# vliu15/speech-masters-thesis

Hardware: AMD Instinct MI355X
Metric: LJSpeech utterances/sec per VQ-VAE train step (higher is better)
Workload: dtype bf16

## Files before the change

include/smt_hip.h:

```cpp
#ifndef SMT_HIP_H
#define SMT_HIP_H

#include <stddef.h>
#include <stdint.h>

#ifdef __cplusplus
extern "C" {
#endif

typedef void* smt_stream_t;

enum { SMT_F32 = 0, SMT_BF16 = 1 };

const char* smt_last_error(void);
int smt_abi_version(void);

size_t smt_vq_prep_bytes(int k_bins, int dim);
int smt_vq_prepare(const float* codebook, int k_bins, int dim, void* prep, size_t prep_bytes, smt_stream_t stream);

size_t smt_vq_forward_workspace_bytes(int64_t n_rows, int k_bins, int dim);
int smt_vq_forward(const float* x, const float* codebook, void* prep, const float* row_mask,
                   int64_t n_rows, int k_bins, int dim,
                   int64_t* idx, float* min_dist, float* x_d, float* sums,
                   void* workspace, size_t workspace_bytes, smt_stream_t stream);
// ... 93 lines not shown
  int64_t bs_x, bs_y, bs_res, bs_act, bs_yact;
  const void* x; const void* w; const float* bias; void* y; void* y_act;
  const void* res; const void* act_grad_src;
  const int* lens_in; const int* lens_out;
  int w_swizzled;
  const void* zero_page;
  const void* x2; const void* w2;
  const float* bias2;
  const int* lens_in2;
  int c_in2, ld_x2;
  int64_t bs_x2;
  const uint32_t* drop_keys_dev;
  int drop_keys_dev_stride;
} smt_conv_desc;
int smt_conv1d_ntc(const smt_conv_desc* desc, smt_stream_t stream);
const char* smt_conv1d_kernel_name(const smt_conv_desc* desc);

size_t smt_conv1d_wgrad_workspace_bytes(const smt_conv_desc* desc);
int smt_conv1d_wgrad(const smt_conv_desc* desc, float* dweight, int64_t stride_out, int64_t stride_in,
                     int64_t stride_tap, const int* tap_map, float* dbias, void* workspace,
                     size_t workspace_bytes, smt_stream_t stream);
int smt_wgrad_reduce_defer(int on, smt_stream_t stream);
const char* smt_conv1d_wgrad_kernel_name(const smt_conv_desc* desc);

size_t smt_conv1x1_bwd_workspace_bytes(const smt_conv_desc* desc);
int smt_conv1x1_bwd(const smt_conv_desc* desc, float* dweight, int64_t stride_out, int64_t stride_in, float* dbias,
                    void* workspace, size_t workspace_bytes, smt_stream_t stream);

size_t smt_conv_k1_bwd_workspace_bytes(int batch, int t);
int smt_conv_k1_bwd(const void* dh, int64_t bs_dh, int ld_dh, const void* x, int64_t bs_x, int ld_x,
                    const void* w_packed_bwd, const void* res, int64_t bs_res, int ld_res, void* dx, int64_t bs_dx,
                    int ld_dx, const int* lens, int batch, int t, const void* zero_page, float* dweight,
                    int64_t stride_out, int64_t stride_in, float* dbias, void* workspace, size_t workspace_bytes,
                    smt_stream_t stream);

int smt_convt4s2(const void* x, int64_t bs_x, int ld_x, const void* w_packed, const float* bias, void* y, int64_t bs_y,
                 int ld_y, const int* lens_in, const int* lens_out, int batch, int t_in, int c_out, const void* zero_page,
                 smt_stream_t stream);
int smt_conv4s2(const void* x, int64_t bs_x, int ld_x, const void* w_packed, const float* bias, void* y, int64_t bs_y,
                int ld_y, const int* lens_in, const int* lens_out, int batch, int t_in, int c_in, const void* zero_page,
                smt_stream_t stream);

int smt_conv_k3gate_fwd(const void* u2, int64_t bs_u2, int ld_u2, const void* x, int64_t bs_x, int ld_x,
                        const void* w3_packed, const void* w1_packed, const float* b3, const float* b1, void* z,
                        int64_t bs_z, int ld_z, void* g, int64_t bs_g, int ld_g, const int* lens, int batch, int t,
                        const void* zero_page, smt_stream_t stream);
// ... 167 lines not shown
```

speech-masters-thesis_amd/csrc/conv_wgrad.hip:

```cpp
#include <algorithm>
#include <cstdlib>

#include "conv_common.h"

namespace smt {

struct WgradArgs {
  const void* x; const void* dy; float* slab;
  const int* lens_in;
  long long x_bs, dy_bs;
  int ldx, ldy;
  int B, Tin, Tout, Ty, Cin, Cout;
  int taps, stride, dil, pad, out_stride, out_offset;
  int rows_per_chunk, chunks_per_batch, nblk_ci, nblk_co, with_bias;
};

template <typename T> struct WTr;
template <> struct WTr<__bf16> {
  static constexpr int R = 128;
  static constexpr int pitch(int ch) { return ch + 32; }
};
template <> struct WTr<float> {
  static constexpr int R = 64;
  static constexpr int pitch(int ch) { return ch + 4; }
// ... 254 lines not shown
          const bf16x8 bfrag = tr_read2(xbase + xoff[j] + k0 * XB, 4 * XB);
          acc[j] = __builtin_amdgcn_mfma_f32_32x32x16_bf16(a, bfrag, acc[j], 0, 0, 0);
        } else if (j == ntaps && bias_plane) {
          acc[j] = __builtin_amdgcn_mfma_f32_32x32x16_bf16(a, ones, acc[j], 0, 0, 0);
        }
      }
    }
    step_end_wait<0>();
  }
  const int planes = ntaps + 1;
  float* out = p.slab + ((size_t)w.cgl * w.nblk + w.blk) * (size_t)planes * CB * CIB;
#pragma unroll
  for (int j = 0; j < NT; ++j) {
    if (j >= planes) break;
#pragma unroll
    for (int e = 0; e < 16; ++e) {
      const int row = wm * 32 + (e & 3) + 8 * (e >> 2) + 4 * hh;
      const int col = wn * 32 + r;
      out[((size_t)j * CB + row) * CIB + col] = acc[j][e];
    }
  }
}

struct ShiftArgs {
  const void* x; const void* dy; float* slab; const int* lens_in;
  long long x_bs, dy_bs;
  int ldx, ldy;
  int B, Tin, Tout, pad, rs;
  int tiles_per_item, tiles_per_wg, n_chunks, nblk_ci, nblk_co, with_bias;
};

#ifndef SMT_WGRAD_STAMP
#define SMT_WGRAD_STAMP 0
#endif
#if SMT_WGRAD_STAMP
__device__ unsigned long long wg_dbg[256 * 8 * 8];
__device__ __forceinline__ unsigned long long wg_stamp() {
  unsigned long long t;
  __builtin_amdgcn_sched_barrier(0);
  asm volatile("s_memtime %0\n\ts_waitcnt lgkmcnt(0)" : "=s"(t) : : "memory");
  __builtin_amdgcn_sched_barrier(0);
  return t;
}
#define WG_SUMS unsigned long long wg_sum[5] = {0, 0, 0, 0, 0}
#define WG_T(var) const unsigned long long var = wg_stamp()
#define WG_ACC(k, a, b) wg_sum[k] += (b) - (a)
#define WG_DUMP do { if (lane == 0 && blockIdx.x < 256) for (int k_ = 0; k_ < 5; ++k_) wg_dbg[(blockIdx.x * 8 + wave) * 8 + k_] += wg_sum[k_]; } while (0)
#else
#define WG_SUMS do {} while (0)
#define WG_T(var) do {} while (0)
#define WG_ACC(k, a, b) do {} while (0)
#define WG_DUMP do {} while (0)
#endif

constexpr int SH_R = 128, SH_XROWS = SH_R + 8, SH_DY = SH_R * 128, SH_X = SH_XROWS * 256, SH_STAGE = SH_DY + SH_X;

template <int NTAPS>
__global__ __launch_bounds__(512) void conv_wgrad_shift_kernel(ShiftArgs p, const __bf16* __restrict__ zero_page) {
  constexpr int CB = 64, CIB = 128, WNC = 4, DYB = CB * 2, XB = CIB * 2, PLANES = NTAPS + 1;
  extern __shared__ __attribute__((aligned(16))) unsigned char smem[];
  const int tid = threadIdx.x, lane = tid & 63;
  const int wave = __builtin_amdgcn_readfirstlane(tid >> 6);
  const int wm = wave / WNC, wn = wave % WNC;
  const int r = lane & 31, hh = lane >> 5;

  const WgBlock w = wgrad_block(p.nblk_ci, p.nblk_co);
  if (w.cgl >= p.n_chunks) return;
  const int co0 = (w.blk / p.nblk_ci) * CB, ci0 = (w.blk % p.nblk_ci) * CIB;
  const int ntiles = p.tiles_per_item * p.B * p.rs;
  const int tile_begin = w.cgl * p.tiles_per_wg;
  const int tile_end = min(ntiles, tile_begin + p.tiles_per_wg);
  const int rs = p.rs;
  const bool bias_plane = p.with_bias && (ci0 == 0);

  f32x16 acc[PLANES];
#pragma unroll
  for (int j = 0; j < PLANES; ++j)
#pragma unroll
    for (int e = 0; e < 16; ++e) acc[j][e] = 0.f;

  constexpr int SH_PIECES = 7;
  constexpr int SH_PPS = 2;
  static_assert(SH_PPS <= NTAPS && SH_PPS * (SH_R / 16) >= SH_PIECES, "the pieces fit the k-loop");
  const unsigned pdy = (unsigned)p.ldy * rs * 2u, pxx = (unsigned)p.ldx * rs * 2u;
  const int dyrow = 8 * wave + (lane >> 3), xrow = 4 * wave + (lane >> 4);
  const unsigned voff_dy = (unsigned)dyrow * pdy + (unsigned)(((lane & 7) ^ swz_dy(dyrow)) << 4);
  const unsigned voff_x = (unsigned)xrow * pxx + (unsigned)(((lane & 15) ^ swz_x(xrow)) << 4);
  const unsigned voff_x6 = (128 + xrow < SH_R + NTAPS - 1) ? voff_x + 128u * pxx : 0x80000000u;
  struct Src { __amdgpu_buffer_rsrc_t rdy, rxx; unsigned sdy, sx; };
  auto item_source = [&](int item, Src& s) {
    const int b = item / rs, cls = item - b * rs;
    const int Tc = (p.Tout - cls + rs - 1) / rs;
    const int len_full = p.lens_in ? min(scalar_load_i32(p.lens_in + b), p.Tin) : p.Tin;
    const int len_in = max(0, (len_full - cls + rs - 1) / rs);
    s.rdy = ws_rsrc(p.dy, ((long long)b * p.dy_bs + (long long)cls * p.ldy + co0) * 2, (unsigned)Tc * pdy);
    s.rxx = ws_rsrc(p.x, ((long long)b * p.x_bs + (long long)cls * p.ldx + ci0) * 2, (unsigned)len_in * pxx);
  };
  auto tile_source = [&](int t0, Src& s) {
    s.sdy = (unsigned)t0 * pdy;
    s.sx = (unsigned)(t0 - p.pad) * pxx;
  };
  auto piece = [&](const Src& s, int i, int buf) {
    unsigned char* base = smem + (size_t)buf * SH_STAGE;
    if (i < 2) ws_dma16(s.rdy, voff_dy + s.sdy + (unsigned)(64 * i) * pdy, base + (wave + 8 * i) * 1024);
    else if (i < 6) ws_dma16(s.rxx, voff_x + s.sx + (unsigned)(32 * (i - 2)) * pxx, base + SH_DY + (wave + 8 * (i - 2)) * 1024);
    else if (wave < 2) ws_dma16(s.rxx, voff_x6 + s.sx, base + SH_DY + (wave + 32) * 1024);
  };

  bf16x8 ones;
#pragma unroll
  for (int e = 0; e < 8; ++e) ones[e] = (__bf16)1.0f;

  const int tg = lane >> 4, tq = (lane & 15) >> 2, tp = lane & 3, thh = tg >> 1;
  const int coly = wm * 32 + 16 * (tg & 1) + 4 * tp, colx = wn * 32 + 16 * (tg & 1) + 4 * tp;
  const int lrow = 8 * thh + tq;
  const int dyoff = lrow * DYB + (((coly >> 3) ^ (((lrow >> 1) & 1) << 2)) << 4) + (coly & 7) * 2;
  const int xoff = SH_DY + lrow * XB + (((colx >> 3) ^ ((lrow & 3) << 2)) << 4) + (colx & 7) * 2;
  typedef unsigned u32x4 __attribute__((ext_vector_type(4)));
  typedef unsigned u32x2 __attribute__((ext_vector_type(2)));
// ... 34 lines not shown
      if (more) item_source(n_item, sn);
    }
    if (!more) sn.rdy = sn.rxx = ws_rsrc(p.x, 0, 0);
    tile_source(n_t0, sn);
    WG_T(c2);
    const unsigned base = lds0 + (unsigned)buf * SH_STAGE;
    Frags fr[2];
    request(fr[0], base, 0);
#pragma unroll
    for (int k0 = 0; k0 < SH_R / 16; ++k0) {
      Frags& f = fr[k0 & 1];
      if (k0 + 1 < SH_R / 16) {
        request(fr[(k0 + 1) & 1], base, k0 + 1);
        lgkm_wait<SH_NREAD>(f.a0, f.a1, f.p0, f.p1, f.q0, f.q1);
      } else {
        lgkm_wait<0>(f.a0, f.a1, f.p0, f.p1, f.q0, f.q1);
      }
      const u32x4 aw = {f.a0[0], f.a0[1], f.a1[0], f.a1[1]};
      const bf16x8 a = __builtin_bit_cast(bf16x8, aw);
      const unsigned w[8] = {f.p0[0], f.p0[1], f.p1[0], f.p1[1], f.q0[0], f.q0[1], f.q1[0], f.q1[1]};
#pragma unroll
      for (int s = 0; s < NTAPS; ++s) {
        const int m = s >> 1;
        u32x4 bw;
        if (s & 1) {
#pragma unroll
          for (int i = 0; i < 4; ++i) bw[i] = __builtin_amdgcn_alignbit(w[m + i + 1], w[m + i], 16);
        } else {
          bw = u32x4{w[m], w[m + 1], w[m + 2], w[m + 3]};
        }
        acc[s] = __builtin_amdgcn_mfma_f32_32x32x16_bf16(a, __builtin_bit_cast(bf16x8, bw), acc[s], 0, 0, 0);
        if (s < SH_PPS && SH_PPS * k0 + s < SH_PIECES) {
          __builtin_amdgcn_sched_barrier(0);
          piece(sn, SH_PPS * k0 + s, buf ^ 1);
          __builtin_amdgcn_sched_barrier(0);
        }
      }
      if (bias_plane && (k0 & 3) == wn) acc[NTAPS] = __builtin_amdgcn_mfma_f32_32x32x16_bf16(a, ones, acc[NTAPS], 0, 0, 0);
    }
    WG_T(c3);
    WG_ACC(0, c0, c1); WG_ACC(1, c1, c2); WG_ACC(2, c2, c3); WG_ACC(4, c0, c0 + 1);
  }
  vm_wait<0>();
  WG_T(c4);
  float* out = p.slab + ((size_t)w.cgl * w.nblk + w.blk) * (size_t)PLANES * CB * CIB;
#pragma unroll
  for (int j = 0; j < PLANES; ++j)
#pragma unroll
    for (int e = 0; e < 16; ++e) {
      const int row = wm * 32 + (e & 3) + 8 * (e >> 2) + 4 * hh;
      out[((size_t)j * CB + row) * CIB + wn * 32 + r] = acc[j][e];
    }
  WG_T(c5);
  WG_ACC(3, c4, c5);
  WG_DUMP;
}

struct ShiftPlan { int rs, pad, tiles_per_item, tiles_per_wg, n_chunks, nblk_co, nblk_ci; };
static bool wgrad_shift_plan(const smt_conv_desc* d, ShiftPlan* pl) {
  static const bool off = getenv("SMT_WGRAD_NO_SHIFT") != nullptr;
  if (off || d->dtype != SMT_BF16 || d->stride != 1 || d->out_stride != 1 || d->out_offset != 0 || !d->zero_page ||
      d->c_in % 128 != 0 || d->c_out % 64 != 0 || d->taps < 3 || d->taps > 9 || !(d->taps & 1) || d->t_in != d->t_out)
    return false;
  int rs = 1, pad = d->padding;
  if (d->dilation > 1) {
    if (d->padding % d->dilation != 0 || d->t_out / d->dilation < class_min_rows()) return false;
    rs = d->dilation; pad = d->padding / d->dilation;
  }
  if (pad < 0 || pad > d->taps - 1) return false;
  const long long tc_max = (d->t_out + rs - 1) / rs;
  const long long span = (tc_max + 2 * SH_R) * rs * 2;
  if (span * d->ld_x >= (1ll << 31) || span * d->ld_y >= (1ll << 31)) return false;
  const int tpi = (int)((tc_max + SH_R - 1) / SH_R);
  const long long ntiles = (long long)tpi * d->batch * rs;
  static const int min_tiles = getenv("SMT_SHIFT_MIN_TILES") ? atoi(getenv("SMT_SHIFT_MIN_TILES")) : 256;
  if (ntiles < min_tiles) return false;
  const int nco = d->c_out / 64, nci = d->c_in / 128;
  static const int min_tpw = getenv("SMT_SHIFT_MIN_TPW") ? atoi(getenv("SMT_SHIFT_MIN_TPW")) : 2;
  const long long chunks_target =
      std::max<long long>(8, std::min<long long>(256 / (nco * nci), ntiles / std::max(1, min_tpw)));
  const int tpw = (int)((ntiles + chunks_target - 1) / chunks_target);
  pl->rs = rs; pl->pad = pad; pl->tiles_per_item = tpi; pl->tiles_per_wg = tpw;
  pl->n_chunks = (int)((ntiles + tpw - 1) / tpw); pl->nblk_co = nco; pl->nblk_ci = nci;
  return true;
}

struct WreduceJob {
  const float* slab; float* dw; float* db;
  long long so, si, sj;
  int n_chunks, nblk, nblk_ci, planes, taps, Cin, Cout, cib, bias_cols;
  int block0;
  int wblocks;
  signed char jmap[16];
};
constexpr int WR_MAXJ = 16;
struct WreduceBatch { int n_jobs, total_blocks; WreduceJob job[WR_MAXJ]; };

__global__ __launch_bounds__(256) void conv_wgrad_reduce_kernel(WreduceBatch bt) {
  __shared__ f32x4 part[4][64];
  int j = 0;
#pragma unroll 1
  for (int k = 1; k < bt.n_jobs; ++k)
    if ((int)blockIdx.x >= bt.job[k].block0) j = k;
  const WreduceJob& p = bt.job[j];
  const int lb = blockIdx.x - p.block0;
  const size_t blk_elems = (size_t)p.planes * 64 * p.cib;
  const size_t cstride = (size_t)p.nblk * blk_elems;
// ... 222 lines not shown
  SMT_CHECK_ARG(d && tap_map, "smt_conv1d_wgrad: null pointer");
  SMT_CHECK_ARG(d->taps >= 1 && d->taps <= WG_MAX_TAPS, "smt_conv1d_wgrad: taps must be in [1, 16]");
  SMT_CHECK_ARG(d->x && d->y && dweight && workspace, "smt_conv1d_wgrad: null pointer");
  SMT_CHECK_ARG(d->dtype == SMT_BF16 || d->dtype == SMT_F32, "smt_conv1d_wgrad: bad dtype");
  const bool bf = d->dtype == SMT_BF16;
  const int epv = bf ? 8 : 4;
  SMT_CHECK_ARG(d->c_in % epv == 0 && d->c_out % epv == 0 && d->ld_x % epv == 0 && d->ld_y % epv == 0,
                "smt_conv1d_wgrad: channels / pitches must keep 16-byte alignment");
  WgradPlan pl;
  wgrad_plan(d, &pl);
  SMT_CHECK_ARG(workspace_bytes >= pl.ws_bytes, "smt_conv1d_wgrad: workspace too small");
  const bool empty = d->batch <= 0 || d->t_out <= 0;
  for (int i = 0; i < pl.n; ++i) {
    const WgradLaunch& l = pl.l[i];
    float* slab = reinterpret_cast<float*>((char*)workspace + l.ws_off);
    float* db = i == 0 ? dbias : nullptr;
    if (l.variant == WG_SHIFT) {
      ShiftArgs a;
      a.x = d->x; a.dy = d->y; a.slab = slab; a.lens_in = d->lens_in;
      a.x_bs = d->bs_x; a.dy_bs = d->bs_y; a.ldx = d->ld_x; a.ldy = d->ld_y;
      a.B = d->batch; a.Tin = d->t_in; a.Tout = d->t_out; a.pad = l.pad; a.rs = pl.sh.rs;
      a.tiles_per_item = pl.sh.tiles_per_item; a.tiles_per_wg = pl.sh.tiles_per_wg; a.n_chunks = l.n_chunks;
      a.nblk_ci = l.nblk_ci; a.nblk_co = l.nblk_co; a.with_bias = db ? 1 : 0;
      const __bf16* zp = (const __bf16*)d->zero_page;
      switch (d->taps) {
        case 3: launch_lds(conv_wgrad_shift_kernel<3>, l.grid, 512, l.lds, stream, a, zp); break;
        case 5: launch_lds(conv_wgrad_shift_kernel<5>, l.grid, 512, l.lds, stream, a, zp); break;
        case 7: launch_lds(conv_wgrad_shift_kernel<7>, l.grid, 512, l.lds, stream, a, zp); break;
        default: launch_lds(conv_wgrad_shift_kernel<9>, l.grid, 512, l.lds, stream, a, zp); break;
      }
      SMT_CHECK_LAUNCH(kWgradName[l.variant]);
    } else if (!empty) {
      SMT_CHECK_ARG(l.lds <= WG_MAX_LDS, "conv_wgrad: tile needs %zu B of LDS", l.lds);
      WgradArgs a;
      a.x = d->x; a.dy = d->y; a.slab = slab; a.lens_in = d->lens_in;
      a.x_bs = d->bs_x; a.dy_bs = d->bs_y; a.ldx = d->ld_x; a.ldy = d->ld_y;
      a.B = d->batch; a.Tin = d->t_in; a.Tout = d->t_out; a.Ty = d->t_y; a.Cin = d->c_in; a.Cout = d->c_out;
      a.taps = l.taps; a.stride = d->stride; a.dil = d->dilation; a.pad = l.pad;
      a.out_stride = d->out_stride; a.out_offset = d->out_offset;
      a.rows_per_chunk = l.rows_per_chunk; a.chunks_per_batch = l.chunks_per_batch;
      a.nblk_ci = l.nblk_ci; a.nblk_co = l.nblk_co; a.with_bias = db ? 1 : 0;
      const bool strided = d->stride > 1;
      const int planes = l.taps + 1;
      const WgradKernel k = l.variant == WG_DMA ? dma_kernel(planes)
                          : bf && l.cib == 128  ? generic_kernel<__bf16, 128, false>(planes)
                          : bf ? (strided ? generic_kernel<__bf16, 64, true>(planes) : generic_kernel<__bf16, 64, false>(planes))
                               : (strided ? generic_kernel<float, 64, true>(planes) : generic_kernel<float, 64, false>(planes));
      launch_lds(k, l.grid, l.variant == WG_DMA ? 512 : l.cib * 4, l.lds, stream, a);
      SMT_CHECK_LAUNCH(kWgradName[l.variant]);
    }
    const int bias_cols = l.variant == WG_SHIFT ? 4 : 1;
    int rc = launch_wgrad_reduce(slab, dweight, db, empty ? 0 : l.n_chunks, l.nblk_co, l.nblk_ci, l.taps, d->c_in, d->c_out,
                                 l.cib, stride_out, stride_in, stride_tap, tap_map + l.j0, stream, bias_cols);
    if (rc) return rc;
  }
  return 0;
}
```

speech-masters-thesis_amd/smt_amd/convops.py:

```python
import contextlib
import ctypes
import os
from dataclasses import dataclass

import torch

from . import native as N
from . import packing
from . import profiler
from .packing import Part

SMT_F32, SMT_BF16 = 0, 1
_DT = {torch.float32: SMT_F32, torch.bfloat16: SMT_BF16}


class ConvDesc(ctypes.Structure):
    _fields_ = [("dtype", ctypes.c_int), ("batch", ctypes.c_int), ("t_in", ctypes.c_int), ("t_out", ctypes.c_int),
                ("t_y", ctypes.c_int), ("c_in", ctypes.c_int), ("c_out", ctypes.c_int), ("taps", ctypes.c_int),
                ("stride", ctypes.c_int), ("dilation", ctypes.c_int), ("padding", ctypes.c_int),
                ("out_stride", ctypes.c_int), ("out_offset", ctypes.c_int), ("act_out", ctypes.c_int),
                ("act_grad", ctypes.c_int), ("site_width", ctypes.c_int), ("ld_x", ctypes.c_int),
                ("ld_y", ctypes.c_int), ("ld_res", ctypes.c_int), ("ld_act", ctypes.c_int), ("ld_yact", ctypes.c_int),
                ("drop_keys", ctypes.c_uint32 * 8), ("drop_thresh16", ctypes.c_uint32), ("drop_scale", ctypes.c_float),
                ("bs_x", ctypes.c_int64), ("bs_y", ctypes.c_int64), ("bs_res", ctypes.c_int64),
                ("bs_act", ctypes.c_int64), ("bs_yact", ctypes.c_int64), ("x", ctypes.c_void_p), ("w", ctypes.c_void_p),
                ("bias", ctypes.c_void_p), ("y", ctypes.c_void_p), ("y_act", ctypes.c_void_p), ("res", ctypes.c_void_p),
                ("act_grad_src", ctypes.c_void_p), ("lens_in", ctypes.c_void_p), ("lens_out", ctypes.c_void_p),
                ("w_swizzled", ctypes.c_int), ("zero_page", ctypes.c_void_p),
                ("x2", ctypes.c_void_p), ("w2", ctypes.c_void_p), ("bias2", ctypes.c_void_p),
                ("lens_in2", ctypes.c_void_p), ("c_in2", ctypes.c_int), ("ld_x2", ctypes.c_int),
                ("bs_x2", ctypes.c_int64), ("drop_keys_dev", ctypes.c_void_p), ("drop_keys_dev_stride", ctypes.c_int)]


@dataclass
class DropSpec:
    p: float
    training: bool
    seed: int = 0
    site: int = 0

    def params(self):
        if not self.training or self.p <= 0.0:
            return 0, 0, 1.0
        return dropout_key(self.seed, self.site), int(round(self.p * 65536.0)), 1.0 / (1.0 - self.p)


def _fmix32(h):
    h &= 0xFFFFFFFF
    h ^= h >> 16
    h = (h * 0x85EBCA6B) & 0xFFFFFFFF
    h ^= h >> 13
    h = (h * 0xC2B2AE35) & 0xFFFFFFFF
    h ^= h >> 16
    return h


# ... 23 lines not shown
    key = (device.type, device.index)
    if key not in _zero_pages:
        _zero_pages[key] = torch.zeros(4096, dtype=torch.uint8, device=device)
    return _zero_pages[key]


def _dma_ok(dtype, c_in, c_out):
    return dtype == torch.bfloat16 and c_in % 128 == 0 and c_out % 128 == 0


def _phases(kernel, stride, padding):
    out = []
    for ph in range(stride):
        taps = [(j, (ph + padding - j) // stride) for j in range(kernel) if (ph + padding - j) % stride == 0]
        taps.sort(key=lambda jt: jt[1])
        offs = [o for _, o in taps]
        assert offs == list(range(offs[0], offs[0] + len(offs))), "phase taps must touch consecutive rows"
        out.append(([j for j, _ in taps], -offs[0]))
    return out


_K3GATE = not bool(int(os.environ.get("SMT_NO_K3GATE", "0")))
_RESAMPLE = not bool(int(os.environ.get("SMT_NO_RESAMPLE", "0")))


def _pack(weight, dtype, n_out, n_in, s_out, s_in, s_tap, tap_map, swizzle=False):
    return packing.pack([Part.dense(weight, n_out, n_in, s_out, s_in, s_tap, tap_map, swizzle)], dtype,
                        (len(tap_map), n_out, n_in))


def _pack_fwd(weight, dtype, swizzle=False):
    c_out, c_in, k = weight.shape
    return _pack(weight, dtype, c_out, c_in, c_in * k, k, 1, range(k), swizzle)


def _pack_bwd(weight, dtype, swizzle=False):
    c_out, c_in, k = weight.shape
    return _pack(weight, dtype, c_in, c_out, k, c_in * k, 1, range(k - 1, -1, -1), swizzle)


def _pack_cat_fwd(weights, dtype, swizzle=False):
    n_in = weights[0].shape[1]
    total = sum(w.shape[0] for w in weights)
    parts, row0 = [], 0
    for w in weights:
        parts.append(Part(w, w.shape[0], n_in, n_in, 1, 1, (0,), bool(swizzle), row0 * n_in, total * n_in, n_in))
# ... 71 lines not shown
    d.batch, d.t_in, d.t_out, d.t_y = x.shape[0], x.shape[1], t_out, (y.shape[1] if t_y is None else t_y)
    d.c_in, d.c_out = c_in, c_out
    d.taps, d.stride, d.dilation, d.padding = taps, stride, dil, pad
    d.out_stride, d.out_offset = out_stride, out_offset
    d.x, d.bs_x, d.ld_x = _geom(x)
    if y is not None:
        d.y, d.bs_y, d.ld_y = _geom(y)
    d.lens_in = _p(lens_in)
    d.drop_scale = 1.0
    return d


def _wgrad(desc, dweight, s_out, s_in, s_tap, tap_map, dbias):
    lib = N.lib()
    desc.zero_page = _p(_zero_page(dweight.device))
    ws_bytes = lib.smt_conv1d_wgrad_workspace_bytes(ctypes.byref(desc))
    ws = N.workspace.get(ws_bytes, dweight.device)
    arr = (ctypes.c_int * len(tap_map))(*tap_map)
    dtype = "bf16" if desc.dtype == SMT_BF16 else "f32"
    name = lib.smt_conv1d_wgrad_kernel_name(ctypes.byref(desc)).decode() + ("_" + _tag(desc) if profiler.DETAIL else "")
    with profiler.region(name, flops=_conv_flops(desc), bound="mfma", dtype=dtype):
        N.check(lib.smt_conv1d_wgrad(ctypes.byref(desc), _p(dweight), s_out, s_in, s_tap, arr, _p(dbias), _p(ws),
                                     ws.numel(), N.stream_ptr()), "smt_conv1d_wgrad")


def _conv1x1_bwd(desc, dweight, s_out, s_in, dbias):
    lib = N.lib()
    ws_bytes = lib.smt_conv1x1_bwd_workspace_bytes(ctypes.byref(desc))
    ws = N.workspace.get(ws_bytes, dweight.device)
    rows = float(desc.batch) * desc.t_out
    name = "conv1x1_bwd" + ("_" + _tag(desc) if profiler.DETAIL else "")
    with profiler.region(name, flops=2 * _conv_flops(desc), nbytes=rows * 3 * desc.c_in * 2, bound="hbm", dtype="bf16"):
        N.check(lib.smt_conv1x1_bwd(ctypes.byref(desc), _p(dweight), s_out, s_in, _p(dbias), _p(ws), ws.numel(),
                                    N.stream_ptr()), "smt_conv1x1_bwd")


def _conv_gate_bwd(dy, g, w_packed_bwd, dx, lens32, dweight, dbias):
    lib = N.lib()
    b, t = g.shape[0], g.shape[1]
    ws = N.workspace.get(lib.smt_conv_gate_bwd_workspace_bytes(b, t), g.device)
    (pdy, bsdy, lddy), (pg, bsg, ldg), (pdx, bsdx, lddx) = _geom(dy), _geom(g), _geom(dx)
    rows = float(b) * t
    with profiler.region("conv_gate_bwd", flops=4.0 * rows * 64 * 64, nbytes=rows * 3 * 64 * 2, bound="hbm", dtype="bf16"):
        N.check(lib.smt_conv_gate_bwd(pdy, bsdy, lddy, pg, bsg, ldg, _p(w_packed_bwd), pdx, bsdx, lddx, _p(lens32), b, t,
                                      _p(_zero_page(g.device)), _p(dweight), dweight.stride(0), dweight.stride(1),
                                      _p(dbias), _p(ws), ws.numel(), N.stream_ptr()), "smt_conv_gate_bwd")
# ... 121 lines not shown
        dx = dw = db = None
        if ctx.needs_input_grad[0]:
            dx = torch.empty(b, t_in, c_in, dtype=x.dtype, device=x.device)
            if stride == 1:
                d = _dgrad_stride1(dy, _pack_bwd(weight, x.dtype), dx, k, dilation, padding)
                d.lens_out = _p(lens32)
                _launch(d, "conv_dgrad", _conv_flops(d), _conv_bytes(d, x.element_size()))
            elif t_in == 2 * t_out and _resample_ok(x.dtype, k, stride, padding, dilation, c_out, c_in):
                wt = _pack(weight, x.dtype, c_in, c_out, k, c_in * k, 1, list(range(k)))
                _resample("convt", "dgrad", dy, wt, None, dx, None, lens32, c_in)
            else:
                for ph, (taps, pad_eff) in enumerate(_phases(k, stride, padding)):
                    n_ph = (t_in - ph + stride - 1) // stride
                    if n_ph <= 0:
                        continue
                    wb = _pack(weight, x.dtype, c_in, c_out, k, c_in * k, 1, taps)
                    d = _base_desc(dy, dx, None, c_out, c_in, len(taps), 1, 1, pad_eff, n_ph, stride, ph)
                    d.w = _p(wb)
                    d.lens_out = _p(lens32)
                    _launch(d, "conv_dgrad", _conv_flops(d), _conv_bytes(d, x.element_size()))
        if ctx.needs_input_grad[1]:
            dw = torch.empty_like(weight)
            db = torch.empty(c_out, dtype=torch.float32, device=x.device)
            d = _base_desc(x, dy, lens32, c_in, c_out, k, stride, dilation, padding, t_out)
            _wgrad(d, dw, c_in * k, k, 1, list(range(k)), db)
            if not has_bias:
                db = None
        return dx, dw, db, (dy if has_res else None), None, None, None, None


def conv1d(x, weight, bias, *, stride=1, padding=0, dilation=1, lens=None, residual=None):
    return _Conv1d.apply(x, weight, bias, residual, lens, stride, padding, dilation)


class _ConvTranspose1d(torch.autograd.Function):
    @staticmethod
    def forward(ctx, x, weight, bias, lens, stride, padding):
        b, t_in, c_in = x.shape
        _, c_out, k = weight.shape
        t_y = (t_in - 1) * stride - 2 * padding + k
        y = torch.empty(b, t_y, c_out, dtype=x.dtype, device=x.device)
        lens32 = _i32(lens)
        fast = _resample_ok(x.dtype, k, stride, padding, 1, c_in, c_out)
        if fast:
            _resample("convt", "fwd", x, _pack(weight, x.dtype, c_out, c_in, k, c_out * k, 1, list(range(k))), bias, y, lens32,
                      None, c_out)
        for ph, (taps, pad_eff) in enumerate(() if fast else _phases(k, stride, padding)):
            n_ph = (t_y - ph + stride - 1) // stride
# ... 300 lines not shown
```

speech-masters-thesis_amd/smt_amd/native.py:

```python
import contextlib
import ctypes
import os
import threading

import torch

_HERE = os.path.dirname(os.path.abspath(__file__))
LIB_PATH = os.environ.get("SMT_HIP_LIB") or os.path.join(_HERE, "libsmt_hip.so")
ABI_VERSION = 10

_lib = None
_lock = threading.Lock()

c_i64 = ctypes.c_int64
c_int = ctypes.c_int
c_f32 = ctypes.c_float
c_u32 = ctypes.c_uint32
c_ptr = ctypes.c_void_p
c_size = ctypes.c_size_t

_SIGNATURES = {
    "smt_last_error": (ctypes.c_char_p, []),
    "smt_abi_version": (c_int, []),
    "smt_vq_forward_workspace_bytes": (c_size, [c_i64, c_int, c_int]),
# ... 2 lines not shown
    "smt_vq_forward": (c_int, [c_ptr, c_ptr, c_ptr, c_ptr, c_i64, c_int, c_int, c_ptr, c_ptr, c_ptr, c_ptr, c_ptr, c_size,
                               c_ptr]),
    "smt_vq_backward": (c_int, [c_ptr, c_ptr, c_ptr, c_ptr, c_ptr, c_ptr, c_i64, c_int, c_ptr, c_ptr]),
    "smt_vq_ema_accumulate_workspace_bytes": (c_size, [c_i64, c_int, c_int]),
    "smt_vq_ema_accumulate": (c_int, [c_ptr, c_ptr, c_ptr, c_i64, c_int, c_int, c_ptr, c_ptr, c_size, c_ptr]),
    "smt_vq_ema_apply": (c_int, [c_ptr, c_ptr, c_ptr, c_ptr, c_ptr, c_f32, c_f32, c_int, c_int, c_ptr, c_ptr, c_size,
                                 c_ptr]),
    "smt_vq_grouped_prep_bytes": (c_size, [c_int, c_int, c_int]),
    "smt_vq_grouped_prepare": (c_int, [c_ptr, c_int, c_int, c_int, c_ptr, c_size, c_ptr]),
    "smt_vq_align_groups": (c_int, [c_ptr, c_ptr, c_int, c_int, c_int, c_int, c_ptr, c_ptr, c_ptr]),
    "smt_vq_grouped_forward_workspace_bytes": (c_size, [c_i64]),
    "smt_vq_grouped_forward": (c_int, [c_ptr, c_ptr, c_ptr, c_ptr, c_ptr, c_i64, c_int, c_int, c_int, c_ptr, c_ptr, c_ptr, c_ptr,
                                       c_ptr, c_ptr, c_size, c_ptr]),
    "smt_vq_grouped_ema_apply": (c_int, [c_ptr, c_ptr, c_ptr, c_ptr, c_ptr, c_f32, c_f32, c_int, c_int, c_int, c_ptr, c_ptr,
                                         c_size, c_ptr]),
    "smt_pack_weight": (c_int, [c_ptr, c_ptr, c_int, c_int, c_int, c_int, c_i64, c_i64, c_i64, c_ptr, c_int, c_ptr]),
    "smt_pack_weights_batched": (c_int, [c_ptr, c_ptr, c_ptr, c_int, c_ptr]),
    "smt_conv1d_ntc": (c_int, [c_ptr, c_ptr]),
    "smt_conv1d_kernel_name": (ctypes.c_char_p, [c_ptr]),
    "smt_conv1d_wgrad_workspace_bytes": (c_size, [c_ptr]),
    "smt_conv1d_wgrad_kernel_name": (ctypes.c_char_p, [c_ptr]),
    "smt_conv1d_wgrad": (c_int, [c_ptr, c_ptr, c_i64, c_i64, c_i64, c_ptr, c_ptr, c_ptr, c_size, c_ptr]),
    "smt_wgrad_reduce_defer": (c_int, [c_int, c_ptr]),
    "smt_conv1x1_bwd_workspace_bytes": (c_size, [c_ptr]),
    "smt_conv1x1_bwd": (c_int, [c_ptr, c_ptr, c_i64, c_i64, c_ptr, c_ptr, c_size, c_ptr]),
    "smt_conv_gate_bwd_workspace_bytes": (c_size, [c_int, c_int]),
    "smt_conv_gate_bwd": (c_int, [c_ptr, c_i64, c_int, c_ptr, c_i64, c_int, c_ptr, c_ptr, c_i64, c_int, c_ptr, c_int,
                                  c_int, c_ptr, c_ptr, c_i64, c_i64, c_ptr, c_ptr, c_size, c_ptr]),
    "smt_conv_k1_bwd_workspace_bytes": (c_size, [c_int, c_int]),
    "smt_conv_k1_bwd": (c_int, [c_ptr, c_i64, c_int, c_ptr, c_i64, c_int, c_ptr, c_ptr, c_i64, c_int, c_ptr, c_i64,
                                c_int, c_ptr, c_int, c_int, c_ptr, c_ptr, c_i64, c_i64, c_ptr, c_ptr, c_size, c_ptr]),
    "smt_convt4s2": (c_int, [c_ptr, c_i64, c_int, c_ptr, c_ptr, c_ptr, c_i64, c_int, c_ptr, c_ptr, c_int, c_int, c_int, c_ptr, c_ptr]),
    "smt_conv4s2": (c_int, [c_ptr, c_i64, c_int, c_ptr, c_ptr, c_ptr, c_i64, c_int, c_ptr, c_ptr, c_int, c_int, c_int, c_ptr, c_ptr]),
    "smt_conv_k3gate_fwd": (c_int, [c_ptr, c_i64, c_int, c_ptr, c_i64, c_int, c_ptr, c_ptr, c_ptr, c_ptr, c_ptr, c_i64, c_int,
                                    c_ptr, c_i64, c_int, c_ptr, c_int, c_int, c_ptr, c_ptr]),
    "smt_gate_mix_fwd": (c_int, [c_ptr, c_ptr, c_int, c_i64, c_int, c_int, c_int, c_int, c_ptr]),
    "smt_gate_mix_bwd": (c_int, [c_ptr, c_ptr, c_ptr, c_int, c_i64, c_int, c_int, c_int, c_int, c_int, c_ptr]),
    "smt_conv_in_fwd": (c_int, [c_ptr, c_ptr, c_ptr, c_ptr, c_ptr, c_int, c_int, c_int, c_int, c_int, c_int, c_int,
                                c_int, c_ptr]),
    "smt_conv_in_wgrad_workspace_bytes": (c_size, [c_int, c_int, c_int]),
    "smt_conv_in_wgrad": (c_int, [c_ptr, c_ptr, c_ptr, c_ptr, c_ptr, c_int, c_int, c_int, c_int, c_int, c_int, c_int,
                                  c_int, c_ptr, c_size, c_ptr]),
    "smt_conv_out_fwd": (c_int, [c_ptr, c_ptr, c_ptr, c_ptr, c_ptr, c_int, c_int, c_int, c_int, c_ptr]),
    "smt_conv_out_bwd_workspace_bytes": (c_size, [c_int, c_int, c_int]),
    "smt_maximum_path": (c_int, [c_ptr, c_ptr, c_int, c_int, c_int, c_f32, c_ptr, c_ptr]),
    "smt_vqtts_distance": (c_int, [c_ptr, c_ptr, c_ptr, c_int, c_int, c_int, c_int, c_ptr]),
# ... 175 lines not shown
```

Before: 520.9.

## Route stride-2 k4 conv weight gradient through masked shifted-fragment kernel

Adds a resample weight-gradient path that views the stride-2 4-tap conv (and transposed conv) as a stride-1 3-tap problem over paired rows, then reuses the shifted-fragment MFMA wgrad kernel. A masked variant skips MFMAs and stores for planes that map to no real tap. A dedicated reduce kernel gathers the slab planes into the weight and bias layout. The aim is to replace the generic strided wgrad with the faster shift kernel. The cost is a larger workspace and extra planes computed for the view. Only the conv (not convt) path is wired in Python.

New measurement: 520.5 (median of 2 runs). About the same (-0.1%).

```diff
diff --git a/include/smt_hip.h b/include/smt_hip.h
--- a/include/smt_hip.h
+++ b/include/smt_hip.h
@@ -139,6 +139,22 @@
                      size_t workspace_bytes, smt_stream_t stream);
 int smt_wgrad_reduce_defer(int on, smt_stream_t stream);
 const char* smt_conv1d_wgrad_kernel_name(const smt_conv_desc* desc);
+
+typedef struct smt_resample_wgrad_desc {
+  int kind;
+  int dtype;
+  const void* x;
+  const void* dy;
+  const int* lens;
+  int64_t bs_x, bs_y;
+  int ld_x, ld_y;
+  int batch, t_x, t_y, c_x, c_y;
+} smt_resample_wgrad_desc;
+int smt_conv_resample_wgrad_eligible(const smt_resample_wgrad_desc* desc);
+size_t smt_conv_resample_wgrad_workspace_bytes(const smt_resample_wgrad_desc* desc);
+int smt_conv_resample_wgrad(const smt_resample_wgrad_desc* desc, float* dweight, int64_t stride_co, int64_t stride_ci,
+                            int64_t stride_tap, float* dbias, void* workspace, size_t workspace_bytes, smt_stream_t stream);
+int smt_conv_resample_wgrad_tap(int kind, int plane, int half, int block);
 
 size_t smt_conv1x1_bwd_workspace_bytes(const smt_conv_desc* desc);
 int smt_conv1x1_bwd(const smt_conv_desc* desc, float* dweight, int64_t stride_out, int64_t stride_in, float* dbias,
diff --git a/speech-masters-thesis_amd/csrc/conv_wgrad.hip b/speech-masters-thesis_amd/csrc/conv_wgrad.hip
--- a/speech-masters-thesis_amd/csrc/conv_wgrad.hip
+++ b/speech-masters-thesis_amd/csrc/conv_wgrad.hip
@@ -300,12 +300,31 @@
   }
 }
 
+enum { RS_CONV = 0, RS_CONVT = 1 };
+
+__host__ __device__ static inline int resample_tap(int kind, int plane, int half, int block) {
+  if (plane < 0 || plane > 2 || half < 0 || half > 1 || block < 0) return -1;
+  if (kind == RS_CONV) {
+    if (block != 0) return -1;
+    const int j = 2 * plane + half - 1;
+    return (j >= 0 && j < 4) ? j : -1;
+  }
+  if (kind == RS_CONVT) {
+    if (block > 3) return -1;
+    const int j = block + 1 - 2 * half - 4 * (plane - 1);
+    return (j >= 0 && j < 4) ? j : -1;
+  }
+  return -1;
+}
+
 struct ShiftArgs {
   const void* x; const void* dy; float* slab; const int* lens_in;
   long long x_bs, dy_bs;
   int ldx, ldy;
   int B, Tin, Tout, pad, rs;
   int tiles_per_item, tiles_per_wg, n_chunks, nblk_ci, nblk_co, with_bias;
+  int x_unit;
+  int rs_kind, rs_cx, rs_cy;
 };
 
 #ifndef SMT_WGRAD_STAMP
@@ -333,7 +352,7 @@
 
 constexpr int SH_R = 128, SH_XROWS = SH_R + 8, SH_DY = SH_R * 128, SH_X = SH_XROWS * 256, SH_STAGE = SH_DY + SH_X;
 
-template <int NTAPS>
+template <int NTAPS, bool MASKED = false>
 __global__ __launch_bounds__(512) void conv_wgrad_shift_kernel(ShiftArgs p, const __bf16* __restrict__ zero_page) {
   constexpr int CB = 64, CIB = 128, WNC = 4, DYB = CB * 2, XB = CIB * 2, PLANES = NTAPS + 1;
   extern __shared__ __attribute__((aligned(16))) unsigned char smem[];
@@ -350,6 +369,14 @@
   const int tile_end = min(ntiles, tile_begin + p.tiles_per_wg);
   const int rs = p.rs;
   const bool bias_plane = p.with_bias && (ci0 == 0);
+  unsigned pmask = ~0u;
+  if constexpr (MASKED) {
+    const int half = ((ci0 + wn * 32) / p.rs_cx) & 1, yblk = (co0 + wm * 32) / p.rs_cy;
+    pmask = 0;
+#pragma unroll
+    for (int s = 0; s < NTAPS; ++s) pmask |= (resample_tap(p.rs_kind, s, half, yblk) >= 0 ? 1u : 0u) << s;
+    pmask = __builtin_amdgcn_readfirstlane(pmask);
+  }
 
   f32x16 acc[PLANES];
 #pragma unroll
@@ -372,7 +399,7 @@
     const int len_full = p.lens_in ? min(scalar_load_i32(p.lens_in + b), p.Tin) : p.Tin;
     const int len_in = max(0, (len_full - cls + rs - 1) / rs);
     s.rdy = ws_rsrc(p.dy, ((long long)b * p.dy_bs + (long long)cls * p.ldy + co0) * 2, (unsigned)Tc * pdy);
-    s.rxx = ws_rsrc(p.x, ((long long)b * p.x_bs + (long long)cls * p.ldx + ci0) * 2, (unsigned)len_in * pxx);
+    s.rxx = ws_rsrc(p.x, ((long long)b * p.x_bs + (long long)cls * p.ldx + ci0) * 2, (unsigned)max(0, len_in * p.x_unit - ci0 * 2));
   };
   auto tile_source = [&](int t0, Src& s) {
     s.sdy = (unsigned)t0 * pdy;
@@ -453,21 +480,23 @@
 #pragma unroll
       for (int s = 0; s < NTAPS; ++s) {
         const int m = s >> 1;
-        u32x4 bw;
-        if (s & 1) {
-#pragma unroll
-          for (int i = 0; i < 4; ++i) bw[i] = __builtin_amdgcn_alignbit(w[m + i + 1], w[m + i], 16);
-        } else {
-          bw = u32x4{w[m], w[m + 1], w[m + 2], w[m + 3]};
+        if (!MASKED || ((pmask >> s) & 1)) {
+          u32x4 bw;
+          if (s & 1) {
+#pragma unroll
+            for (int i = 0; i < 4; ++i) bw[i] = __builtin_amdgcn_alignbit(w[m + i + 1], w[m + i], 16);
+          } else {
+            bw = u32x4{w[m], w[m + 1], w[m + 2], w[m + 3]};
+          }
+          acc[s] = __builtin_amdgcn_mfma_f32_32x32x16_bf16(a, __builtin_bit_cast(bf16x8, bw), acc[s], 0, 0, 0);
         }
-        acc[s] = __builtin_amdgcn_mfma_f32_32x32x16_bf16(a, __builtin_bit_cast(bf16x8, bw), acc[s], 0, 0, 0);
         if (s < SH_PPS && SH_PPS * k0 + s < SH_PIECES) {
           __builtin_amdgcn_sched_barrier(0);
           piece(sn, SH_PPS * k0 + s, buf ^ 1);
           __builtin_amdgcn_sched_barrier(0);
         }
       }
-      if (bias_plane && (k0 & 3) == wn) acc[NTAPS] = __builtin_amdgcn_mfma_f32_32x32x16_bf16(a, ones, acc[NTAPS], 0, 0, 0);
+      if (bias_plane && (MASKED ? wn == 0 : (k0 & 3) == wn)) acc[NTAPS] = __builtin_amdgcn_mfma_f32_32x32x16_bf16(a, ones, acc[NTAPS], 0, 0, 0);
     }
     WG_T(c3);
     WG_ACC(0, c0, c1); WG_ACC(1, c1, c2); WG_ACC(2, c2, c3); WG_ACC(4, c0, c0 + 1);
@@ -476,21 +505,42 @@
   WG_T(c4);
   float* out = p.slab + ((size_t)w.cgl * w.nblk + w.blk) * (size_t)PLANES * CB * CIB;
 #pragma unroll
-  for (int j = 0; j < PLANES; ++j)
+  for (int j = 0; j < PLANES; ++j) {
+    if (MASKED && j < NTAPS && !((pmask >> j) & 1)) continue;
 #pragma unroll
     for (int e = 0; e < 16; ++e) {
       const int row = wm * 32 + (e & 3) + 8 * (e >> 2) + 4 * hh;
       out[((size_t)j * CB + row) * CIB + wn * 32 + r] = acc[j][e];
     }
+  }
   WG_T(c5);
   WG_ACC(3, c4, c5);
   WG_DUMP;
 }
 
 struct ShiftPlan { int rs, pad, tiles_per_item, tiles_per_wg, n_chunks, nblk_co, nblk_ci; };
+static bool shift_tiling(long long tc_max, int rs, int batch, long long ld_x, long long ld_y, int nco, int nci, ShiftPlan* pl) {
+  const long long span = (tc_max + 2 * SH_R) * rs * 2;
+  if (span * ld_x >= (1ll << 31) || span * ld_y >= (1ll << 31)) return false;
+  const int tpi = (int)((tc_max + SH_R - 1) / SH_R);
+  const long long ntiles = (long long)tpi * batch * rs;
+  static const int min_tiles = getenv("SMT_SHIFT_MIN_TILES") ? atoi(getenv("SMT_SHIFT_MIN_TILES")) : 256;
+  if (ntiles < min_tiles) return false;
+  static const int min_tpw = getenv("SMT_SHIFT_MIN_TPW") ? atoi(getenv("SMT_SHIFT_MIN_TPW")) : 2;
+  const long long chunks_target =
+      std::max<long long>(8, std::min<long long>(256 / (nco * nci), ntiles / std::max(1, min_tpw)));
+  const int tpw = (int)((ntiles + chunks_target - 1) / chunks_target);
+  pl->tiles_per_item = tpi; pl->tiles_per_wg = tpw;
+  pl->n_chunks = (int)((ntiles + tpw - 1) / tpw); pl->nblk_co = nco; pl->nblk_ci = nci;
+  return true;
+}
+
+static bool shift_switched_off() {
+  static const bool off = getenv("SMT_WGRAD_NO_SHIFT") != nullptr;
+  return off;
+}
 static bool wgrad_shift_plan(const smt_conv_desc* d, ShiftPlan* pl) {
-  static const bool off = getenv("SMT_WGRAD_NO_SHIFT") != nullptr;
-  if (off || d->dtype != SMT_BF16 || d->stride != 1 || d->out_stride != 1 || d->out_offset != 0 || !d->zero_page ||
+  if (shift_switched_off() || d->dtype != SMT_BF16 || d->stride != 1 || d->out_stride != 1 || d->out_offset != 0 || !d->zero_page ||
       d->c_in % 128 != 0 || d->c_out % 64 != 0 || d->taps < 3 || d->taps > 9 || !(d->taps & 1) || d->t_in != d->t_out)
     return false;
   int rs = 1, pad = d->padding;
@@ -499,21 +549,8 @@
     rs = d->dilation; pad = d->padding / d->dilation;
   }
   if (pad < 0 || pad > d->taps - 1) return false;
-  const long long tc_max = (d->t_out + rs - 1) / rs;
-  const long long span = (tc_max + 2 * SH_R) * rs * 2;
-  if (span * d->ld_x >= (1ll << 31) || span * d->ld_y >= (1ll << 31)) return false;
-  const int tpi = (int)((tc_max + SH_R - 1) / SH_R);
-  const long long ntiles = (long long)tpi * d->batch * rs;
-  static const int min_tiles = getenv("SMT_SHIFT_MIN_TILES") ? atoi(getenv("SMT_SHIFT_MIN_TILES")) : 256;
-  if (ntiles < min_tiles) return false;
-  const int nco = d->c_out / 64, nci = d->c_in / 128;
-  static const int min_tpw = getenv("SMT_SHIFT_MIN_TPW") ? atoi(getenv("SMT_SHIFT_MIN_TPW")) : 2;
-  const long long chunks_target =
-      std::max<long long>(8, std::min<long long>(256 / (nco * nci), ntiles / std::max(1, min_tpw)));
-  const int tpw = (int)((ntiles + chunks_target - 1) / chunks_target);
-  pl->rs = rs; pl->pad = pad; pl->tiles_per_item = tpi; pl->tiles_per_wg = tpw;
-  pl->n_chunks = (int)((ntiles + tpw - 1) / tpw); pl->nblk_co = nco; pl->nblk_ci = nci;
-  return true;
+  pl->rs = rs; pl->pad = pad;
+  return shift_tiling((d->t_out + rs - 1) / rs, rs, d->batch, d->ld_x, d->ld_y, d->c_out / 64, d->c_in / 128, pl);
 }
 
 struct WreduceJob {
@@ -782,6 +819,8 @@
       a.B = d->batch; a.Tin = d->t_in; a.Tout = d->t_out; a.pad = l.pad; a.rs = pl.sh.rs;
       a.tiles_per_item = pl.sh.tiles_per_item; a.tiles_per_wg = pl.sh.tiles_per_wg; a.n_chunks = l.n_chunks;
       a.nblk_ci = l.nblk_ci; a.nblk_co = l.nblk_co; a.with_bias = db ? 1 : 0;
+      a.x_unit = d->ld_x * pl.sh.rs * 2;
+      a.rs_kind = a.rs_cx = a.rs_cy = 0;
       const __bf16* zp = (const __bf16*)d->zero_page;
       switch (d->taps) {
         case 3: launch_lds(conv_wgrad_shift_kernel<3>, l.grid, 512, l.lds, stream, a, zp); break;
@@ -816,3 +855,173 @@
   }
   return 0;
 }
+
+namespace smt {
+
+struct ResampleReduce {
+  const float* slab; float* dw; float* db;
+  long long so, si, sj;
+  int n_chunks, nblk, nblk_ci, Cx, Cy, yblocks, wblocks;
+  int nsrc;
+  signed char plane[4][2], half[4][2], yblk[4][2];
+};
+
+__global__ __launch_bounds__(256) void conv_resample_reduce_kernel(ResampleReduce p) {
+  __shared__ f32x4 part[4][64];
+  constexpr size_t blk_elems = (size_t)4 * 64 * 128;
+  const size_t cstride = (size_t)p.nblk * blk_elems;
+  const int lb = blockIdx.x;
+  if (lb < p.wblocks) {
+    const int o = threadIdx.x & 63, sl = threadIdx.x >> 6;
+    const int cx4 = p.Cx >> 2;
+    const int total4 = 4 * p.Cy * cx4;
+    const int e4 = lb * 64 + o;
+    const bool live = e4 < total4;
+    f32x4 s = {0.f, 0.f, 0.f, 0.f};
+    int ci = 0, co = 0, j = 0;
+    if (live) {
+      ci = (e4 % cx4) * 4; co = (e4 / cx4) % p.Cy; j = e4 / (cx4 * p.Cy);
+      const float* src[2] = {nullptr, nullptr};
+      for (int q = 0; q < p.nsrc; ++q) {
+        const int civ = p.half[j][q] * p.Cx + ci, cov = p.yblk[j][q] * p.Cy + co;
+        const int blk = (cov / 64) * p.nblk_ci + civ / 128;
+        src[q] = p.slab + (size_t)blk * blk_elems + ((size_t)p.plane[j][q] * 64 + (cov % 64)) * 128 + (civ % 128);
+      }
+      for (int c = sl; c < p.n_chunks; c += 4) {
+        s += *reinterpret_cast<const f32x4*>(src[0] + (size_t)c * cstride);
+        if (p.nsrc > 1) s += *reinterpret_cast<const f32x4*>(src[1] + (size_t)c * cstride);
+      }
+    }
+    part[sl][o] = s;
+    __syncthreads();
+    if (sl == 0 && live) {
+      f32x4 t = part[0][o];
+#pragma unroll
+      for (int k = 1; k < 4; ++k) t += part[k][o];
+      float* dst = p.dw + co * p.so + ci * p.si + j * p.sj;
+      dst[0] = t[0]; dst[p.si] = t[1]; dst[2 * p.si] = t[2]; dst[3 * p.si] = t[3];
+    }
+  } else {
+    float* part1 = reinterpret_cast<float*>(&part[0][0]);
+    const int o = threadIdx.x & 31, sl = threadIdx.x >> 5;
+    const int co = (lb - p.wblocks) * 32 + o;
+    const bool live = co < p.Cy && p.db != nullptr;
+    float s = 0.f;
+    if (live) {
+      for (int c = sl; c < p.n_chunks; c += 8) {
+        for (int yb = 0; yb < p.yblocks; ++yb) {
+          const int cov = yb * p.Cy + co;
+          const float* q = p.slab + (size_t)c * cstride + (size_t)((cov / 64) * p.nblk_ci) * blk_elems + ((size_t)3 * 64 + (cov % 64)) * 128;
+          s += q[0];
+        }
+      }
+    }
+    part1[sl * 32 + o] = s;
+    __syncthreads();
+    if (sl == 0 && live) {
+      float t = part1[o];
+#pragma unroll
+      for (int k = 1; k < 8; ++k) t += part1[k * 32 + o];
+      p.db[co] = t;
+    }
+  }
+}
+
+struct ResamplePlan { ShiftPlan sh; int t_view, ldx_v, ldy_v; size_t ws_bytes; };
+
+static const char* resample_plan(const smt_resample_wgrad_desc* d, ResamplePlan* pl) {
+  if (!d) return "null descriptor";
+  if (d->kind != RS_CONV && d->kind != RS_CONVT) return "kind must be 0 (conv) or 1 (transposed)";
+  if (d->dtype != SMT_BF16) return "bf16 only";
+  if (shift_switched_off()) return "the shifted-fragment kernel is switched off (SMT_WGRAD_NO_SHIFT)";
+  if ((d->c_x != 64 && d->c_x != 128) || (d->c_y != 64 && d->c_y != 128)) return "channels must be 64 or 128";
+  if (!d->x || !d->dy) return "null operand";
+  if (d->batch <= 0 || d->t_x <= 0 || (d->t_x & 1)) return "t_x must be even and positive";
+  const bool convt = d->kind == RS_CONVT;
+  if (d->t_y != (convt ? 2ll * d->t_x : d->t_x / 2)) return "dy must have exactly t_x / 2 (conv) or 2 t_x (transposed) rows";
+  if (d->ld_x != d->c_x) return "the row pitch of x must equal its channel count";
+  if (convt ? d->ld_y != d->c_y : (d->ld_y < d->c_y || d->ld_y % 8 != 0)) return "the row pitch of dy does not fit the view";
+  if (((uintptr_t)d->x | (uintptr_t)d->dy) % 16 != 0 || d->bs_x % 8 != 0 || d->bs_y % 8 != 0) return "operands must keep 16-byte alignment";
+  pl->t_view = d->t_x / 2;
+  pl->ldx_v = 2 * d->c_x;
+  pl->ldy_v = convt ? 4 * d->c_y : d->ld_y;
+  pl->sh.rs = 1; pl->sh.pad = 1;
+  const int nco = (convt ? 4 * d->c_y : d->c_y) / 64, nci = pl->ldx_v / 128;
+  if (!shift_tiling(pl->t_view, 1, d->batch, pl->ldx_v, pl->ldy_v, nco, nci, &pl->sh))
+    return "an item spans 2^31 bytes or the viewed problem has too few 128-row tiles";
+  if (!convt) {
+    smt_conv_desc g = {};
+    g.dtype = SMT_BF16; g.batch = d->batch; g.t_in = d->t_x; g.t_out = g.t_y = pl->t_view; g.c_in = d->c_x; g.c_out = d->c_y;
+    g.taps = 4; g.stride = 2; g.dilation = 1; g.padding = 1; g.out_stride = 1;
+    const WgradLaunch l = wgrad_group_plan(&g, 0, 4);
+    pl->sh.tiles_per_wg = l.rows_per_chunk / SH_R;
+    pl->sh.tiles_per_item = l.chunks_per_batch * pl->sh.tiles_per_wg;
+    pl->sh.n_chunks = l.n_chunks;
+    const long long padded = (long long)(pl->sh.tiles_per_item + 2) * SH_R * 2;
+    if (padded * pl->ldx_v >= (1ll << 31) || padded * pl->ldy_v >= (1ll << 31)) return "an item padded to whole chunks spans 2^31 bytes";
+  }
+  pl->ws_bytes = (size_t)pl->sh.n_chunks * nco * nci * 4 * 64 * 128 * sizeof(float);
+  return nullptr;
+}
+
+}
+
+extern "C" int smt_conv_resample_wgrad_tap(int kind, int plane, int half, int block) { return resample_tap(kind, plane, half, block); }
+
+extern "C" int smt_conv_resample_wgrad_eligible(const smt_resample_wgrad_desc* d) {
+  ResamplePlan pl;
+  return resample_plan(d, &pl) == nullptr ? 1 : 0;
+}
+
+extern "C" size_t smt_conv_resample_wgrad_workspace_bytes(const smt_resample_wgrad_desc* d) {
+  ResamplePlan pl;
+  return resample_plan(d, &pl) == nullptr ? pl.ws_bytes : 0;
+}
+
+extern "C" int smt_conv_resample_wgrad(const smt_resample_wgrad_desc* d, float* dweight, int64_t stride_co, int64_t stride_ci,
+                                       int64_t stride_tap, float* dbias, void* workspace, size_t workspace_bytes,
+                                       smt_stream_t stream_) {
+  hipStream_t stream = (hipStream_t)stream_;
+  ResamplePlan pl;
+  const char* why = resample_plan(d, &pl);
+  SMT_CHECK_ARG(why == nullptr, "smt_conv_resample_wgrad: not eligible: %s", why);
+  SMT_CHECK_ARG(dweight && workspace, "smt_conv_resample_wgrad: null pointer");
+  SMT_CHECK_ARG(workspace_bytes >= pl.ws_bytes, "smt_conv_resample_wgrad: workspace too small");
+  const bool convt = d->kind == RS_CONVT;
+  ShiftArgs a;
+  a.x = d->x; a.dy = d->dy; a.slab = reinterpret_cast<float*>(workspace); a.lens_in = d->lens;
+  a.x_bs = d->bs_x; a.dy_bs = d->bs_y; a.ldx = pl.ldx_v; a.ldy = pl.ldy_v;
+  a.B = d->batch; a.Tin = d->t_x; a.Tout = pl.t_view; a.pad = 1; a.rs = 1;
+  a.tiles_per_item = pl.sh.tiles_per_item; a.tiles_per_wg = pl.sh.tiles_per_wg; a.n_chunks = pl.sh.n_chunks;
+  a.nblk_ci = pl.sh.nblk_ci; a.nblk_co = pl.sh.nblk_co; a.with_bias = dbias ? 1 : 0;
+  a.x_unit = d->c_x * 2;
+  const unsigned grid = (unsigned)(8 * ((a.n_chunks + 7) / 8) * a.nblk_co * a.nblk_ci);
+  a.rs_kind = d->kind; a.rs_cx = d->c_x; a.rs_cy = d->c_y;
+  launch_lds(conv_wgrad_shift_kernel<3, true>, grid, 512, (size_t)2 * SH_STAGE, stream, a, (const __bf16*)nullptr);
+  SMT_CHECK_LAUNCH("conv_wgrad_shift:resample");
+
+  ResampleReduce r;
+  r.slab = a.slab; r.dw = dweight; r.db = dbias;
+  r.so = stride_co; r.si = stride_ci; r.sj = stride_tap;
+  r.n_chunks = a.n_chunks; r.nblk = a.nblk_co * a.nblk_ci; r.nblk_ci = a.nblk_ci; r.Cx = d->c_x; r.Cy = d->c_y;
+  r.yblocks = convt ? 4 : 1;
+  r.nsrc = 0;
+  for (int j = 0; j < 4; ++j) {
+    int n = 0;
+    for (int half = 0; half < 2; ++half)
+      for (int plane = 0; plane < 3; ++plane)
+        for (int blk = 0; blk < r.yblocks; ++blk)
+          if (resample_tap(d->kind, plane, half, blk) == j && n < 2) {
+            r.plane[j][n] = (signed char)plane; r.half[j][n] = (signed char)half; r.yblk[j][n] = (signed char)blk;
+            ++n;
+          }
+    SMT_CHECK_ARG(n == (convt ? 2 : 1), "smt_conv_resample_wgrad: tap map is inconsistent");
+    for (int q = n; q < 2; ++q) r.plane[j][q] = r.half[j][q] = r.yblk[j][q] = 0;
+    r.nsrc = n;
+  }
+  r.wblocks = (4 * d->c_y * (d->c_x / 4) + 63) / 64;
+  const unsigned rblocks = (unsigned)(r.wblocks + (dbias ? (d->c_y + 31) / 32 : 0));
+  conv_resample_reduce_kernel<<<rblocks, 256, 0, stream>>>(r);
+  SMT_CHECK_LAUNCH("conv_resample_reduce");
+  return 0;
+}
diff --git a/speech-masters-thesis_amd/smt_amd/convops.py b/speech-masters-thesis_amd/smt_amd/convops.py
--- a/speech-masters-thesis_amd/smt_amd/convops.py
+++ b/speech-masters-thesis_amd/smt_amd/convops.py
@@ -32,6 +32,13 @@
                 ("bs_x2", ctypes.c_int64), ("drop_keys_dev", ctypes.c_void_p), ("drop_keys_dev_stride", ctypes.c_int)]
 
 
+class ResampleWgradDesc(ctypes.Structure):
+    _fields_ = [("kind", ctypes.c_int), ("dtype", ctypes.c_int), ("x", ctypes.c_void_p), ("dy", ctypes.c_void_p),
+                ("lens", ctypes.c_void_p), ("bs_x", ctypes.c_int64), ("bs_y", ctypes.c_int64), ("ld_x", ctypes.c_int),
+                ("ld_y", ctypes.c_int), ("batch", ctypes.c_int), ("t_x", ctypes.c_int), ("t_y", ctypes.c_int),
+                ("c_x", ctypes.c_int), ("c_y", ctypes.c_int)]
+
+
 @dataclass
 class DropSpec:
     p: float
@@ -101,6 +108,7 @@
 
 _K3GATE = not bool(int(os.environ.get("SMT_NO_K3GATE", "0")))
 _RESAMPLE = not bool(int(os.environ.get("SMT_NO_RESAMPLE", "0")))
+_RESAMPLE_WGRAD = not bool(int(os.environ.get("SMT_NO_RESAMPLE_WGRAD", "0")))
 
 
 def _pack(weight, dtype, n_out, n_in, s_out, s_in, s_tap, tap_map, swizzle=False):
@@ -218,6 +226,32 @@
     with profiler.region(name, flops=_conv_flops(desc), bound="mfma", dtype=dtype):
         N.check(lib.smt_conv1d_wgrad(ctypes.byref(desc), _p(dweight), s_out, s_in, s_tap, arr, _p(dbias), _p(ws),
                                      ws.numel(), N.stream_ptr()), "smt_conv1d_wgrad")
+
+
+RESAMPLE_CONV, RESAMPLE_CONVT = 0, 1
+
+
+def _resample_wgrad_desc(kind, x, dy, lens32):
+    if not _RESAMPLE_WGRAD or x.dtype not in _DT or dy.dtype != x.dtype:
+        return None
+    d = ResampleWgradDesc()
+    d.kind, d.dtype = kind, _DT[x.dtype]
+    d.x, d.bs_x, d.ld_x = _geom(x)
+    d.dy, d.bs_y, d.ld_y = _geom(dy)
+    d.lens = _p(lens32)
+    d.batch, d.t_x, d.t_y, d.c_x, d.c_y = x.shape[0], x.shape[1], dy.shape[1], x.shape[2], dy.shape[2]
+    return d if N.lib().smt_conv_resample_wgrad_eligible(ctypes.byref(d)) else None
+
+
+def _resample_wgrad(d, dweight, s_co, s_ci, s_tap, dbias):
+    lib = N.lib()
+    ws = N.workspace.get(lib.smt_conv_resample_wgrad_workspace_bytes(ctypes.byref(d)), dweight.device)
+    rows_y = float(d.batch) * min(d.t_x, d.t_y)
+    name = "conv_wgrad_shift:resample" + (f"_{'conv' if d.kind == RESAMPLE_CONV else 'convt'}_c{d.c_x}x{d.c_y}" if profiler.DETAIL else "")
+    with profiler.region(name, flops=2.0 * d.c_x * d.c_y * 4 * rows_y,
+                         nbytes=2.0 * d.batch * (d.t_x * d.c_x + d.t_y * d.c_y), bound="mfma", dtype="bf16"):
+        N.check(lib.smt_conv_resample_wgrad(ctypes.byref(d), _p(dweight), s_co, s_ci, s_tap, _p(dbias), _p(ws), ws.numel(),
+                                            N.stream_ptr()), "smt_conv_resample_wgrad")
 
 
 def _conv1x1_bwd(desc, dweight, s_out, s_in, dbias):
@@ -385,8 +419,12 @@
         if ctx.needs_input_grad[1]:
             dw = torch.empty_like(weight)
             db = torch.empty(c_out, dtype=torch.float32, device=x.device)
-            d = _base_desc(x, dy, lens32, c_in, c_out, k, stride, dilation, padding, t_out)
-            _wgrad(d, dw, c_in * k, k, 1, list(range(k)), db)
+            rd = _resample_wgrad_desc(RESAMPLE_CONV, x, dy, lens32) if (k, stride, padding, dilation) == (4, 2, 1, 1) else None
+            if rd is not None:
+                _resample_wgrad(rd, dw, c_in * k, k, 1, db)
+            else:
+                d = _base_desc(x, dy, lens32, c_in, c_out, k, stride, dilation, padding, t_out)
+                _wgrad(d, dw, c_in * k, k, 1, list(range(k)), db)
             if not has_bias:
                 db = None
         return dx, dw, db, (dy if has_res else None), None, None, None, None
diff --git a/speech-masters-thesis_amd/smt_amd/native.py b/speech-masters-thesis_amd/smt_amd/native.py
--- a/speech-masters-thesis_amd/smt_amd/native.py
+++ b/speech-masters-thesis_amd/smt_amd/native.py
@@ -48,6 +48,10 @@
     "smt_conv1d_wgrad_kernel_name": (ctypes.c_char_p, [c_ptr]),
     "smt_conv1d_wgrad": (c_int, [c_ptr, c_ptr, c_i64, c_i64, c_i64, c_ptr, c_ptr, c_ptr, c_size, c_ptr]),
     "smt_wgrad_reduce_defer": (c_int, [c_int, c_ptr]),
+    "smt_conv_resample_wgrad_eligible": (c_int, [c_ptr]),
+    "smt_conv_resample_wgrad_workspace_bytes": (c_size, [c_ptr]),
+    "smt_conv_resample_wgrad": (c_int, [c_ptr, c_ptr, c_i64, c_i64, c_i64, c_ptr, c_ptr, c_size, c_ptr]),
+    "smt_conv_resample_wgrad_tap": (c_int, [c_int, c_int, c_int, c_int]),
     "smt_conv1x1_bwd_workspace_bytes": (c_size, [c_ptr]),
     "smt_conv1x1_bwd": (c_int, [c_ptr, c_ptr, c_i64, c_i64, c_ptr, c_ptr, c_size, c_ptr]),
     "smt_conv_gate_bwd_workspace_bytes": (c_size, [c_int, c_int]),
```
